# NVIDIA/retinanet-examples

Hardware: AMD Instinct MI355X
Metric: images/sec end-to-end (incl. decode+NMS), RN50FPN 800px bs=8 (higher is better)
Workload: dtype bf16; 1 GPU; ResNet50FPN bf16 inference, bs=8 per GPU at 800x1280, HIP decode x5 + NMS; global_batch=8, parallelism=replicas x1 (no data-path collective), entry=Model.forward (eval), postproc=fused

## Files before the change

include/odtk_hip.h:

```cpp
#ifndef ODTK_HIP_H
#define ODTK_HIP_H

#include <stddef.h>
#include <stdint.h>

#ifdef __cplusplus
extern "C" {
#endif

#define ODTK_OK                0
#define ODTK_ERR_INVALID      -1
#define ODTK_ERR_WORKSPACE    -2
#define ODTK_ERR_HIP          -3
#define ODTK_ERR_UNSUPPORTED  -4

#define ODTK_MAX_LEVELS    6
#define ODTK_MAX_ANCHORS   32
#define ODTK_ATSS_MAX_TOPK 16
#define ODTK_MAX_TOP_N     16384
#define ODTK_MAX_NMS_COUNT 7680
#define ODTK_MAX_NMS_COUNT_SCRATCH (1 << 22)
#define ODTK_MAX_NMS_DETECTIONS 2048

#define ODTK_F32   0
// ... 174 lines not shown
                       const odtk_image_t *images, int max_pixels, const void *src, size_t src_bytes, const int32_t *tables,
                       size_t tables_len, const void *norm_table, void *out, int height, int width, int dtype, void *workspace,
                       size_t workspace_bytes, void *stream);
int odtk_gemm_init(const char *hipblaslt_path);
size_t odtk_gemm_plan_export(char *text, size_t capacity);
int odtk_gemm_plan_import(const char *text);
int odtk_gemm_plan_pin_misses(void);
#define ODTK_GEMM_ORIGIN_TIMED   0
#define ODTK_GEMM_ORIGIN_PINNED  1
#define ODTK_GEMM_ORIGIN_CAPTURE 2
int odtk_debug_gemm_candidates(size_t m, int n, int k, int dtype, int relu, int residual, size_t workspace_size,
                               int *indices, int capacity);
void odtk_gemm_plan_clear(void);
int odtk_gemm_last_solution(int *origin);
int odtk_gemm_bias_act(void *y, const void *x, const void *w, const float *bias, const void *residual,
                       size_t m, int n, int k, int dtype, int relu,
                       void *workspace, size_t workspace_size, void *stream);
int odtk_bottleneck_seam(void *out, void *z, const void *y2, const void *skip, const void *w3, const float *b3, const void *w1,
                         const float *b1, size_t m, int c_in, int c_mid, int c_next, int dtype, void *stream);

int odtk_tower_conv3x3(void *y, const void *x, const void *w, const void *bias, int batch_size, int height, int width, int c_in,
                       int c_out, int dtype, int relu, void *stream);
int odtk_debug_tower_conv_variant(int variant);

int odtk_snap_to_anchors(int batch_size, const float *targets, int n_max, const float *anchors,
                         int num_anchors, int num_classes, int height, int width, int stride,
                         float iou_background, float iou_foreground,
                         float *cls_target, float *box_target, float *depth, void *stream);

typedef struct odtk_snap_level {
  const float *anchors;
  float *cls_target;
  float *box_target;
  float *depth;
  int32_t height, width, stride, pad_;
} odtk_snap_level_t;
int odtk_snap_to_anchors_levels(int batch_size, const float *targets, int n_max, int n_levels,
                                const odtk_snap_level_t *levels, int num_anchors, int num_classes,
                                float iou_background, float iou_foreground, void *stream);

int odtk_atss_assign_levels(int batch_size, const float *targets, int n_max, int n_levels,
                            const odtk_snap_level_t *levels, int num_anchors, int num_classes, int topk,
                            void *workspace, size_t workspace_size, void *stream);

struct odtk_loss_level;
int odtk_tal_assign_levels(int batch_size, const float *targets, int n_max, int n_levels,
// ... 124 lines not shown
```

retinanet-examples_amd/csrc/engine.hip:

```cpp
#include <cstring>

#include "runtime.hpp"
#include "epilogue.hpp"
#include "gemm_lt.hpp"
#include "seam.hpp"
#include "tower_conv.hpp"

namespace {

constexpr int kStreamCapMax = 65536, kStreamWideBit = 1 << 20;
std::atomic<int> g_stream_tuning{0};

inline int stream_tuning() { return g_stream_tuning.load(std::memory_order_relaxed); }

inline uint64_t stream_grid(uint64_t blocks, uint64_t own_cap, int tuning) {
  const uint64_t cap = (tuning & (kStreamWideBit - 1)) ? static_cast<uint64_t>(tuning & (kStreamWideBit - 1)) : own_cap;
  return blocks > cap ? cap : blocks;
}

struct BiasActPlan {
  bool fast;
  uint32_t blocks;
  uint32_t vpr;
  uint64_t n_vec;
// ... 66 lines not shown

template <typename T, int N2>
int seam_launch(const void *y2, const void *skip, const void *w3, const float *b3, const void *w1, const float *b1, void *out, void *z,
                uint64_t m, hipStream_t stream) {
  constexpr size_t lds = odtk::seam_lds_bytes<N2>();
  const int rc = allow_dynamic_lds(reinterpret_cast<const void *>(&odtk::bottleneck_seam_kernel<T, N2>), lds, "bottleneck_seam_kernel LDS");
  if (rc != ODTK_OK) return rc;
  int device = 0, cus = 0;
  ODTK_HIP_TRY(hipGetDevice(&device));
  ODTK_HIP_TRY(hipDeviceGetAttribute(&cus, hipDeviceAttributeMultiprocessorCount, device));
  constexpr uint64_t per_group = odtk::kSeamThreads / 64 * 32;
  uint64_t blocks = (m + per_group - 1) / per_group;
  const uint64_t resident = static_cast<uint64_t>(cus > 0 ? cus : 1) * (160 * 1024 / lds);
  if (blocks > resident) blocks = resident;
  timed_launch(ODTK_KERNEL_SEAM, odtk::bottleneck_seam_kernel<T, N2>, dim3(static_cast<unsigned>(blocks)), dim3(odtk::kSeamThreads), lds, stream,
               static_cast<const uint16_t *>(y2), static_cast<const uint16_t *>(skip), static_cast<const uint16_t *>(w3), b3,
               static_cast<const uint16_t *>(w1), b1, static_cast<uint16_t *>(out), static_cast<uint16_t *>(z), m);
  ODTK_HIP_TRY(hipGetLastError());
  return ODTK_OK;
}

std::atomic<int> g_tower_variant{1};

template <typename T, bool kRelu, int kForm>
int tower_conv_launch(void *y, const void *x, const void *w, const void *bias, uint32_t m, uint32_t height, uint32_t width, bool remap,
                      hipStream_t stream) {
  const int rc = allow_dynamic_lds(reinterpret_cast<const void *>(&odtk::tower_conv3x3_kernel<T, kRelu, kForm>), odtk::tower::kLdsBytes,
                                   "tower_conv3x3_kernel LDS");
  if (rc != ODTK_OK) return rc;
  const uint32_t tiles = (m + odtk::tower::kTilePixels - 1) / odtk::tower::kTilePixels;
  timed_launch(ODTK_KERNEL_TOWER_CONV, odtk::tower_conv3x3_kernel<T, kRelu, kForm>, dim3(tiles), dim3(odtk::tower::kThreads),
               odtk::tower::kLdsBytes, stream, static_cast<const unsigned char *>(x), static_cast<const unsigned char *>(w),
               static_cast<const uint16_t *>(bias), static_cast<unsigned char *>(y), m, height, width, odtk::fastdiv_make(width),
               odtk::fastdiv_make(height * width), remap ? 1u : 0u);
  ODTK_HIP_TRY(hipGetLastError());
  return ODTK_OK;
}

template <typename T>
int tower_conv_typed(void *y, const void *x, const void *w, const void *bias, uint32_t m, uint32_t h, uint32_t wd, bool relu, int variant,
                     hipStream_t s) {
  const bool remap = variant & 1;
  if (variant & 2) return relu ? tower_conv_launch<T, true, 0>(y, x, w, bias, m, h, wd, remap, s) : tower_conv_launch<T, false, 0>(y, x, w, bias, m, h, wd, remap, s);
  return relu ? tower_conv_launch<T, true, 1>(y, x, w, bias, m, h, wd, remap, s) : tower_conv_launch<T, false, 1>(y, x, w, bias, m, h, wd, remap, s);
}

}

extern "C" {

int odtk_debug_tower_conv_variant(int variant) {
  if (variant < -1 || variant > 3) return ODTK_ERR_INVALID;
  return variant < 0 ? g_tower_variant.load() : g_tower_variant.exchange(variant);
}

int odtk_debug_stream_tuning(int grid_cap, int pool_wide_index) {
  if (grid_cap < -1 || grid_cap > kStreamCapMax || pool_wide_index < -1 || pool_wide_index > 1) return ODTK_ERR_INVALID;
  int was = g_stream_tuning.load(std::memory_order_relaxed), now;
  do {
    now = (grid_cap < 0 ? was & (kStreamWideBit - 1) : grid_cap) | (pool_wide_index < 0 ? was & kStreamWideBit : pool_wide_index ? kStreamWideBit : 0);
  } while (!g_stream_tuning.compare_exchange_weak(was, now, std::memory_order_relaxed));
  return ODTK_OK;
}

int odtk_debug_stream_tuning_get(int out[2]) {
  if (!out) return ODTK_ERR_INVALID;
  const int tuning = stream_tuning();
// ... 11 lines not shown
  out[1] = p.blocks;
  out[2] = static_cast<unsigned>(p.stride);
  out[3] = p.trips > 0xffffffffull ? 0xffffffffu : static_cast<unsigned>(p.trips);
  return ODTK_OK;
}

int odtk_tower_conv3x3(void *y, const void *x, const void *w, const void *bias, int batch_size, int height, int width, int c_in, int c_out,
                       int dtype, int relu, void *stream) {
  if (!y || !x || !w || !bias || batch_size <= 0 || height <= 0 || width <= 0 || c_in <= 0 || c_out <= 0) return ODTK_ERR_INVALID;
  if (y == x) return ODTK_ERR_INVALID;
  if (dtype != ODTK_BF16 && dtype != ODTK_F16) return ODTK_ERR_UNSUPPORTED;
  if (c_in != static_cast<int>(odtk::tower::kChannels) || c_out != static_cast<int>(odtk::tower::kChannels)) return ODTK_ERR_UNSUPPORTED;
  if ((reinterpret_cast<uintptr_t>(y) | reinterpret_cast<uintptr_t>(x) | reinterpret_cast<uintptr_t>(w) | reinterpret_cast<uintptr_t>(bias)) & 15u)
    return ODTK_ERR_INVALID;
  const uint64_t m = static_cast<uint64_t>(batch_size) * static_cast<uint64_t>(height) * static_cast<uint64_t>(width);
  if (m * odtk::tower::kPixelBytes >= (1ull << 31)) return ODTK_ERR_UNSUPPORTED;
  hipStream_t s = static_cast<hipStream_t>(stream);
  const int variant = g_tower_variant.load(std::memory_order_relaxed);
  if (dtype == ODTK_BF16)
    return tower_conv_typed<odtk::BF16>(y, x, w, bias, static_cast<uint32_t>(m), static_cast<uint32_t>(height), static_cast<uint32_t>(width),
                                        relu != 0, variant, s);
  return tower_conv_typed<odtk::F16>(y, x, w, bias, static_cast<uint32_t>(m), static_cast<uint32_t>(height), static_cast<uint32_t>(width),
                                      relu != 0, variant, s);
}

int odtk_bottleneck_seam(void *out, void *z, const void *y2, const void *skip, const void *w3, const float *b3, const void *w1,
                         const float *b1, size_t m, int c_in, int c_mid, int c_next, int dtype, void *stream) {
  if (!out || !z || !y2 || !skip || !w3 || !b3 || !w1 || !b1 || c_in <= 0 || c_mid <= 0 || c_next <= 0) return ODTK_ERR_INVALID;
  if (out == z || out == y2 || out == skip || z == y2 || z == skip) return ODTK_ERR_INVALID;
  if (dtype != ODTK_BF16 && dtype != ODTK_F16) return ODTK_ERR_UNSUPPORTED;
  if (c_in != odtk::kSeamCin || c_mid != odtk::kSeamCmid || (c_next != 64 && c_next != 128)) return ODTK_ERR_UNSUPPORTED;
  if ((reinterpret_cast<uintptr_t>(out) | reinterpret_cast<uintptr_t>(z) | reinterpret_cast<uintptr_t>(y2) | reinterpret_cast<uintptr_t>(skip) |
       reinterpret_cast<uintptr_t>(w3) | reinterpret_cast<uintptr_t>(w1)) & 15u)
    return ODTK_ERR_INVALID;
  if ((reinterpret_cast<uintptr_t>(b3) | reinterpret_cast<uintptr_t>(b1)) & 3u) return ODTK_ERR_INVALID;
  if (m > (1ull << 40)) return ODTK_ERR_INVALID;
  if (m == 0) return ODTK_OK;
  hipStream_t s = static_cast<hipStream_t>(stream);
  if (dtype == ODTK_BF16)
    return c_next == 64 ? seam_launch<odtk::BF16, 64>(y2, skip, w3, b3, w1, b1, out, z, m, s)
                        : seam_launch<odtk::BF16, 128>(y2, skip, w3, b3, w1, b1, out, z, m, s);
  return c_next == 64 ? seam_launch<odtk::F16, 64>(y2, skip, w3, b3, w1, b1, out, z, m, s)
                      : seam_launch<odtk::F16, 128>(y2, skip, w3, b3, w1, b1, out, z, m, s);
}

int odtk_bias_act(void *y, const float *bias, const void *residual, size_t n_pixels, int channels, int dtype,
// ... 147 lines not shown
```

retinanet-examples_amd/csrc/tower_conv.hpp:

```cpp
#pragma once

#include "common.hpp"
#include "seam.hpp"
#include "tower_conv_layout.hpp"

namespace odtk {

typedef float tower_f32x4 __attribute__((ext_vector_type(4)));

__device__ __attribute__((aligned(16))) uint32_t tower_zero_block[4];

template <typename T>
__device__ __forceinline__ tower_f32x4 tower_mfma(vuint4 a, vuint4 b, tower_f32x4 c) {
  if constexpr (std::is_same_v<T, BF16>)
    return __builtin_amdgcn_mfma_f32_16x16x32_bf16(__builtin_bit_cast(seam_bf16x8, a), __builtin_bit_cast(seam_bf16x8, b), c, 0, 0, 0);
  else
    return __builtin_amdgcn_mfma_f32_16x16x32_f16(__builtin_bit_cast(seam_f16x8, a), __builtin_bit_cast(seam_f16x8, b), c, 0, 0, 0);
}

template <typename T>
__device__ __forceinline__ seam_f32x16 tower_mfma32(vuint4 a, vuint4 b, seam_f32x16 c) {
  if constexpr (std::is_same_v<T, BF16>)
    return __builtin_amdgcn_mfma_f32_32x32x16_bf16(__builtin_bit_cast(seam_bf16x8, a), __builtin_bit_cast(seam_bf16x8, b), c, 0, 0, 0);
  else
    return __builtin_amdgcn_mfma_f32_32x32x16_f16(__builtin_bit_cast(seam_f16x8, a), __builtin_bit_cast(seam_f16x8, b), c, 0, 0, 0);
}

__device__ __forceinline__ void tower_glds16(const unsigned char *src, unsigned char *lds_wave_base) {
  __builtin_amdgcn_global_load_lds((const __attribute__((address_space(1))) void *)src,
                                   (__attribute__((address_space(3))) void *)lds_wave_base, 16, 0, 0);
}

template <typename T, bool kRelu, int kForm>
__global__ __launch_bounds__(tower::kThreads) void tower_conv3x3_kernel(const unsigned char *__restrict__ x, const unsigned char *__restrict__ w,
                                                                        const uint16_t *__restrict__ bias, unsigned char *__restrict__ y,
                                                                        uint32_t m, uint32_t height, uint32_t width, FastDiv by_w,
                                                                        FastDiv by_hw, uint32_t remap) {
  using namespace tower;
  extern __shared__ __attribute__((aligned(1024))) unsigned char tower_lds[];

  const uint32_t tid = threadIdx.x, lane = tid & 63u;
  const uint32_t wave = __builtin_amdgcn_readfirstlane(tid >> 6);
  uint32_t tile = blockIdx.x;
  if (remap) {
    const uint32_t nwg = gridDim.x, q = nwg >> 3, r = nwg & 7u, xcd = tile & 7u;
    tile = (xcd < r ? xcd * (q + 1u) : r * (q + 1u) + (xcd - r) * q) + (tile >> 3);
  }

  const uint32_t chunk_bytes = piece_chunk(tid) * 16u;
  int32_t a_base[4];
  uint32_t a_mask[4];
#pragma unroll
  for (uint32_t i = 0; i < 4; ++i) {
    const uint32_t p = tile * kTilePixels + piece_row(i, tid);
    a_base[i] = 0;
    a_mask[i] = 0u;
    if (p < m) {
      const Pixel px = pixel_of(p, by_w, by_hw);
      a_base[i] = static_cast<int32_t>(p * kPixelBytes + chunk_bytes);
      a_mask[i] = tap_mask(px.y, px.x, height, width);
// ... 17 lines not shown
  };

  const uint32_t wr = wave >> 2, wc = wave & 3u;
  using Acc = std::conditional_t<kForm == 0, tower_f32x4[4][8], seam_f32x16[2][4]>;
  Acc acc;
  if constexpr (kForm == 0) {
#pragma unroll
    for (int n = 0; n < 4; ++n)
#pragma unroll
      for (int b = 0; b < 8; ++b) acc[n][b] = tower_f32x4{0.0f, 0.0f, 0.0f, 0.0f};
  } else {
#pragma unroll
    for (int n = 0; n < 2; ++n)
#pragma unroll
      for (int b = 0; b < 4; ++b)
#pragma unroll
        for (int e = 0; e < 16; ++e) acc[n][b][e] = 0.0f;
  }
  uint32_t f[4];
  if constexpr (kForm == 0) {
    f[0] = frag_addr(0, 0, lane); f[1] = frag_addr(0, 1, lane); f[2] = f[3] = 0u;
  } else {
#pragma unroll
    for (uint32_t s = 0; s < 4; ++s) f[s] = frag32_addr(0, s, lane);
  }
  const uint32_t x_frag = wr * 128u * kRowBytes, w_frag = kOperandBytes + wc * 64u * kRowBytes;

  auto compute = [&](const unsigned char *buf) {
    if constexpr (kForm == 0) {
#pragma unroll
      for (uint32_t kk = 0; kk < 2; ++kk) {
        vuint4 wf[4], xf[8];
#pragma unroll
        for (uint32_t n = 0; n < 4; ++n) wf[n] = *reinterpret_cast<const vuint4 *>(buf + w_frag + n * 16u * kRowBytes + f[kk]);
#pragma unroll
        for (uint32_t b = 0; b < 8; ++b) xf[b] = *reinterpret_cast<const vuint4 *>(buf + x_frag + b * 16u * kRowBytes + f[kk]);
#pragma unroll
        for (uint32_t n = 0; n < 4; ++n)
#pragma unroll
          for (uint32_t b = 0; b < 8; ++b) acc[n][b] = tower_mfma<T>(wf[n], xf[b], acc[n][b]);
      }
    } else {
#pragma unroll
      for (uint32_t s = 0; s < 4; ++s) {
        vuint4 wf[2], xf[4];
#pragma unroll
        for (uint32_t n = 0; n < 2; ++n) wf[n] = *reinterpret_cast<const vuint4 *>(buf + w_frag + n * 32u * kRowBytes + f[s]);
// ... 33 lines not shown
      }
  } else {
#pragma unroll
    for (uint32_t n = 0; n < 2; ++n)
#pragma unroll
      for (uint32_t b = 0; b < 4; ++b)
#pragma unroll
        for (uint32_t g = 0; g < 4; ++g) {
          const uint32_t at = out_addr(acc32_pixel(wr * 4u + b, lane), acc32_channel(wc * 2u + n, lane, 4u * g));
          uint2 v;
          v.x = seam_pack2<T>(acc[n][b][4 * g], acc[n][b][4 * g + 1]);
          v.y = seam_pack2<T>(acc[n][b][4 * g + 2], acc[n][b][4 * g + 3]);
          *reinterpret_cast<uint2 *>(tower_lds + at) = v;
        }
  }
  __syncthreads();
  const uint32_t pixel0 = tid >> 5, chunk = out_chunk(pixel0, tid & 31u);
  float bias8[8];
  {
    const vuint4 bv = *reinterpret_cast<const vuint4 *>(bias + chunk * 8u);
#pragma unroll
    for (int e = 0; e < 8; ++e) bias8[e] = seam_unpack<T>(bv[e >> 1], e & 1);
  }
#pragma unroll 4
  for (uint32_t it = 0; it < 16; ++it) {
    const uint32_t pixel = it * 16u + pixel0, p = tile * kTilePixels + pixel;
    const vuint4 v = *reinterpret_cast<const vuint4 *>(tower_lds + (it * kThreads + tid) * 16u);
    vuint4 r;
#pragma unroll
    for (int d = 0; d < 4; ++d) {
      float o[2];
#pragma unroll
      for (int e = 0; e < 2; ++e) {
        const float s = seam_unpack<T>(v[d], e) + bias8[2 * d + e];
        o[e] = kRelu ? (s > 0.0f ? s : (s != s ? s : 0.0f)) : s;
      }
      r[d] = seam_pack2<T>(o[0], o[1]);
    }
    if (p < m) *reinterpret_cast<vuint4 *>(y + static_cast<size_t>(p) * kPixelBytes + chunk * 16u) = r;
  }
}

}
```

retinanet-examples_amd/csrc/tower_conv_layout.hpp:

```cpp
#pragma once

#include "fastdiv.hpp"

namespace odtk {
namespace tower {

constexpr uint32_t kThreads = 512;
constexpr uint32_t kTilePixels = 256, kChannels = 256, kBK = 64, kTaps = 9;
constexpr uint32_t kKTiles = kTaps * kChannels / kBK;
constexpr uint32_t kRowBytes = kBK * 2, kOperandBytes = 256 * kRowBytes;
constexpr uint32_t kBufferBytes = 2 * kOperandBytes;
constexpr uint32_t kLdsBytes = 2 * kBufferBytes;
constexpr uint32_t kPixelBytes = kChannels * 2;

ODTK_HD uint32_t swizzle(uint32_t row, uint32_t chunk) { return chunk ^ ((row >> 1) & 7u); }

ODTK_HD uint32_t piece_dst(uint32_t i, uint32_t tid) { return (i * kThreads + tid) * 16u; }
ODTK_HD uint32_t piece_wave_base(uint32_t i, uint32_t wave) { return (i * kThreads + wave * 64u) * 16u; }
ODTK_HD uint32_t piece_row(uint32_t i, uint32_t tid) { return i * 64u + (tid >> 3); }
ODTK_HD uint32_t piece_chunk(uint32_t tid) { return swizzle(tid >> 3, tid & 7u); }

ODTK_HD uint32_t frag_row(uint32_t block, uint32_t lane) { return block * 16u + (lane & 15u); }
ODTK_HD uint32_t frag_chunk(uint32_t kk, uint32_t lane) { return kk * 4u + (lane >> 4); }
ODTK_HD uint32_t frag_addr(uint32_t block, uint32_t kk, uint32_t lane) {
  const uint32_t row = frag_row(block, lane);
  return row * kRowBytes + (swizzle(row, frag_chunk(kk, lane)) << 4);
}

ODTK_HD uint32_t frag32_row(uint32_t block, uint32_t lane) { return block * 32u + (lane & 31u); }
ODTK_HD uint32_t frag32_chunk(uint32_t step, uint32_t lane) { return (step >> 1) * 4u + 2u * (lane >> 5) + (step & 1u); }
ODTK_HD uint32_t frag32_addr(uint32_t block, uint32_t step, uint32_t lane) {
  const uint32_t row = frag32_row(block, lane);
  return row * kRowBytes + (swizzle(row, frag32_chunk(step, lane)) << 4);
}

ODTK_HD uint32_t ktile_tap(uint32_t kt) { return kt >> 2; }
ODTK_HD uint32_t ktile_channel(uint32_t kt) { return (kt & 3u) * kBK; }
ODTK_HD int32_t tap_pixel_offset(uint32_t tap, uint32_t width) {
  return (static_cast<int32_t>(tap / 3u) - 1) * static_cast<int32_t>(width) + (static_cast<int32_t>(tap % 3u) - 1);
}

struct Pixel { uint32_t n, y, x; };
ODTK_HD Pixel pixel_of(uint32_t p, const FastDiv &by_w, const FastDiv &by_hw) {
  Pixel q;
  uint32_t rem;
  q.n = fastdivmod(p, by_hw, &rem);
  q.y = fastdivmod(rem, by_w, &q.x);
  return q;
}

ODTK_HD uint32_t tap_mask(uint32_t y, uint32_t x, uint32_t height, uint32_t width) {
  const uint32_t rows = (y > 0u ? 1u : 0u) | 2u | (y + 1u < height ? 4u : 0u);
  const uint32_t cols = (x > 0u ? 1u : 0u) | 2u | (x + 1u < width ? 4u : 0u);
  uint32_t mask = 0u;
  for (uint32_t kh = 0; kh < 3u; ++kh)
    if ((rows >> kh) & 1u) mask |= cols << (3u * kh);
  return mask;
}

ODTK_HD uint32_t out_chunk(uint32_t pixel, uint32_t chunk) { return (chunk & ~7u) | ((chunk ^ pixel) & 7u); }
ODTK_HD uint32_t out_addr(uint32_t pixel, uint32_t channel) {
  return pixel * kPixelBytes + out_chunk(pixel, channel >> 3) * 16u + (channel & 4u) * 2u;
}
ODTK_HD uint32_t acc_channel(uint32_t nb, uint32_t lane, uint32_t reg) { return nb * 16u + (lane >> 4) * 4u + reg; }
ODTK_HD uint32_t acc_pixel(uint32_t mb, uint32_t lane) { return mb * 16u + (lane & 15u); }
ODTK_HD uint32_t acc32_channel(uint32_t nb, uint32_t lane, uint32_t reg) { return nb * 32u + (reg & 3u) + 8u * (reg >> 2) + 4u * (lane >> 5); }
ODTK_HD uint32_t acc32_pixel(uint32_t mb, uint32_t lane) { return mb * 32u + (lane & 31u); }

}
}
```

retinanet-examples_amd/odtk/_C.py:

```python
import ctypes
import threading
import os

import torch

_LIB_PATH = os.environ.get('ODTK_HIP_LIBRARY') or os.path.join(os.path.dirname(os.path.abspath(__file__)), 'libodtk_hip.so')

OK, ERR_INVALID, ERR_WORKSPACE, ERR_HIP, ERR_UNSUPPORTED = 0, -1, -2, -3, -4
F32, BF16, F16 = 0, 1, 2
FLAG_ROTATED, FLAG_LOGITS, FLAG_ROTATED_NMS_FIXED_ANGLE = 1, 2, 4
MAX_LEVELS, MAX_ANCHORS, MAX_TOP_N, MAX_NMS_COUNT, MAX_NMS_COUNT_SCRATCH = 6, 32, 16384, 7680, 1 << 22
MAX_CONCAT_PARTS = 8
MAX_TILES = 64
MAX_OPTIM_TENSORS, OPTIM_CHUNK = 64, 4096
SOFT_NMS_LINEAR, SOFT_NMS_GAUSSIAN = 1, 2
MATRIX_NMS_LINEAR, MATRIX_NMS_GAUSSIAN = 1, 2
MAX_MATRIX_NMS_PRE = 4096
ATSS_MAX_TOPK = 16
BOX_LOSS_IOU, BOX_LOSS_GIOU, BOX_LOSS_DIOU = 1, 2, 3
BOX_LOSS_KINDS = {'iou': BOX_LOSS_IOU, 'giou': BOX_LOSS_GIOU, 'diou': BOX_LOSS_DIOU}
ROTATED_BOX_LOSS_PROBIOU, ROTATED_BOX_LOSS_KLD = 1, 2
ROTATED_BOX_LOSS_KINDS = {'probiou': ROTATED_BOX_LOSS_PROBIOU, 'kld': ROTATED_BOX_LOSS_KLD}
CLS_LOSS_QFL, CLS_LOSS_VFL = 1, 2
CLS_LOSS_KINDS = {'qfl': CLS_LOSS_QFL, 'vfl': CLS_LOSS_VFL}
# ... 158 lines not shown
    'odtk_soft_nms': (ctypes.c_int, [ctypes.c_int, _vpp, _vpp, ctypes.c_int, _sz, ctypes.c_int, ctypes.c_float, ctypes.c_int,
                                     ctypes.c_float, ctypes.c_float, ctypes.c_uint32, _vp, _sz, _vp]),
    'odtk_matrix_nms': (ctypes.c_int, [ctypes.c_int, _vpp, _vpp, ctypes.c_int, _sz, ctypes.c_int, ctypes.c_int, ctypes.c_int,
                                       ctypes.c_float, ctypes.c_float, ctypes.c_uint32, _vp, _sz, _vp]),
    'odtk_box_vote': (ctypes.c_int, [ctypes.c_int, _vpp, _vp, _vp, _sz, ctypes.c_int, ctypes.c_float, ctypes.c_uint32, _vp]),
    'odtk_concat_candidates': (ctypes.c_int, [ctypes.c_int, ctypes.c_int, ctypes.POINTER(Candidates), _vpp, ctypes.c_uint32, _vp]),
    'odtk_tile_images': (ctypes.c_int, [_vp, _vp] + [ctypes.c_int] * 7 + [ctypes.POINTER(Tile), ctypes.c_int, ctypes.c_int, _vp]),
    'odtk_merge_tile_candidates': (ctypes.c_int, [ctypes.c_int, ctypes.POINTER(Tile), _vpp, _vpp, _sz] + [ctypes.c_int] * 6 +
                                   [ctypes.c_float, ctypes.c_uint32, _vp]),
    'odtk_gemm_init': (ctypes.c_int, [ctypes.c_char_p]),
    'odtk_gemm_plan_export': (ctypes.c_size_t, [ctypes.c_char_p, ctypes.c_size_t]),
    'odtk_gemm_plan_import': (ctypes.c_int, [ctypes.c_char_p]),
    'odtk_gemm_plan_pin_misses': (ctypes.c_int, []),
    'odtk_debug_gemm_candidates': (ctypes.c_int, [ctypes.c_size_t] + [ctypes.c_int] * 5 + [ctypes.c_size_t, ctypes.POINTER(ctypes.c_int),
                                                  ctypes.c_int]),
    'odtk_gemm_plan_clear': (None, []),
    'odtk_gemm_last_solution': (ctypes.c_int, [ctypes.POINTER(ctypes.c_int)]),
    'odtk_gemm_bias_act': (ctypes.c_int, [ctypes.c_void_p, ctypes.c_void_p, ctypes.c_void_p, ctypes.c_void_p, ctypes.c_void_p,
                                          ctypes.c_size_t, ctypes.c_int, ctypes.c_int, ctypes.c_int, ctypes.c_int,
                                          ctypes.c_void_p, ctypes.c_size_t, ctypes.c_void_p]),
    'odtk_bottleneck_seam': (ctypes.c_int, [ctypes.c_void_p] * 8 + [ctypes.c_size_t] + [ctypes.c_int] * 4 + [ctypes.c_void_p]),
    'odtk_tower_conv3x3': (ctypes.c_int, [ctypes.c_void_p] * 4 + [ctypes.c_int] * 7 + [ctypes.c_void_p]),
    'odtk_debug_tower_conv_variant': (ctypes.c_int, [ctypes.c_int]),
    'odtk_profile_collect': (ctypes.c_int, [ctypes.POINTER(ctypes.c_double), ctypes.POINTER(ctypes.c_int)]),
}

KERNEL_NAMES = ('prefilter_scan_kernel', 'select_decode_kernel', 'nms_kernel', 'iou_pairs_kernel', 'bias_act_kernel',
                'snap_to_anchors_kernel', 'gemm_bias_act', 'retina_loss_kernel', 'select_hist_kernel', 'select_filter_kernel',
                'nms_first_round_kernel', 'rotated_sup_matrix_kernel', 'bias_act_maxpool_kernel', 'upsample_nearest2x_kernel',
                'stem_pack_kernel', 'loss_reduce_kernel', 'atss_stats_kernel', 'bottleneck_seam_kernel', 'tower_conv3x3_kernel')
traffic_count = False
traffic_bytes = {}


def _count(name, nbytes):
    if traffic_count:
        traffic_bytes[name] = traffic_bytes.get(name, 0) + int(nbytes)


_lib = None


def library():
    global _lib
    if _lib is None:
        if not os.path.isfile(_LIB_PATH):
# ... 994 lines not shown


def tower_conv3x3(x, weight, bias, relu=True):
    if not x.is_cuda or x.dim() != 4 or x.dtype not in (torch.bfloat16, torch.float16):
        raise RuntimeError('tower_conv3x3: x must be a 4-d CUDA tensor of bfloat16/float16')
    b, c, h, w = x.shape
    n = weight.shape[0]
    if (weight.dim() != 4 or tuple(weight.shape[1:]) != (c, 3, 3) or weight.dtype != x.dtype or weight.device != x.device
            or not weight.is_contiguous(memory_format=torch.channels_last)):
        raise RuntimeError('tower_conv3x3: weight must be a channels_last [Cout, %d, 3, 3] tensor of x.dtype' % c)
    if not x.is_contiguous(memory_format=torch.channels_last):
        raise RuntimeError('tower_conv3x3: x must be channels_last')
    if bias.dtype != x.dtype or bias.numel() != n or bias.device != x.device or not bias.is_contiguous():
        raise RuntimeError('tower_conv3x3: bias must be a dense vector of length Cout of x.dtype')
    y = torch.empty((b, n, h, w), dtype=x.dtype, device=x.device, memory_format=torch.channels_last)
    if y.numel() == 0:
        return y
    _launch(library().odtk_tower_conv3x3, 'tower_conv3x3', x.device, y.data_ptr(), x.data_ptr(), weight.data_ptr(), bias.data_ptr(),
            b, h, w, c, n, _DTYPES[x.dtype], 1 if relu else 0)
    _count('tower_conv3x3_kernel', (x.numel() + y.numel()) * x.element_size())
    return y


_CONV_LIB_PATH = os.path.join(os.path.dirname(os.path.abspath(__file__)), 'libodtk_conv.so')
_conv_lib = []


def conv_library():
    if not _conv_lib:
        lib = None
        if os.path.isfile(_CONV_LIB_PATH) and not os.environ.get('ODTK_NO_CONV_LIBRARY'):
            lib = ctypes.CDLL(_CONV_LIB_PATH)
            lib.odtk_conv_bias_act.restype = ctypes.c_int
            lib.odtk_conv_bias_act.argtypes = [ctypes.c_void_p] * 4 + [ctypes.c_int] * 13 + [ctypes.c_void_p]
            lib.odtk_conv_bias_act_pads.restype = ctypes.c_int
            lib.odtk_conv_bias_act_pads.argtypes = [ctypes.c_void_p] * 4 + [ctypes.c_int] * 15 + [ctypes.c_void_p]
            lib.odtk_conv_bias_act_strided.restype = ctypes.c_int
            lib.odtk_conv_bias_act_strided.argtypes = ([ctypes.c_void_p] * 4 + [ctypes.c_int] * 13 + [ctypes.c_longlong] * 6 +
                                                       [ctypes.c_int] * 2 + [ctypes.c_void_p])
            lib.odtk_conv_last_plan.restype = ctypes.c_char_p
            lib.odtk_conv_last_plan.argtypes = []
            lib.odtk_conv_instance_count.restype = ctypes.c_int
            lib.odtk_conv_instance_count.argtypes = [ctypes.c_int]
            lib.odtk_conv_plan_export.restype = ctypes.c_size_t
            lib.odtk_conv_plan_export.argtypes = [ctypes.c_char_p, ctypes.c_size_t]
            lib.odtk_conv_plan_import.restype = ctypes.c_int
# ... 240 lines not shown
```

retinanet-examples_amd/odtk/fused.py:

```python
import hashlib
import json
import os
import threading

import torch
import torch.nn as nn
import torch.nn.functional as F

from . import _C
from . import box as box_ops
from .backbones.resnet import BasicBlock, Bottleneck


_PLAN_LOCK = threading.Lock()
_TLS = threading.local()


def _planning():
    return getattr(_TLS, 'planning', False)


def _key_str(key):
    kind, shape = ('only', key[1:]) if key and key[0] == 'only' else ('act', key)
    return kind + ':' + 'x'.join(str(int(v)) for v in shape)
# ... 44 lines not shown
    shelf_w, row_y, row_h, cursor = None, 0, 0, shelf_x
    for h, w in shapes[1:]:
        if shelf_w is None:
            shelf_w = w
        elif cursor + w > shelf_x + shelf_w and row_y + row_h + gutter + h <= height:
            row_y, row_h, cursor = row_y + row_h + gutter, 0, shelf_x
        origins.append((row_y, cursor))
        shelf_w = max(shelf_w, cursor + w - shelf_x)
        row_h = max(row_h, h)
        cursor += w + gutter
    return ((max(y + h for (y, _), (h, _) in zip(origins, shapes)), max(x + w for (_, x), (_, w) in zip(origins, shapes))), origins)


def _window(x):
    return (x.dim() == 4 and x.shape[1] > 1 and x.stride(1) == 1 and x.stride(3) >= x.shape[1]
            and all(v % 8 == 0 for v in (x.stride(0), x.stride(2), x.stride(3))))


class _Conv(nn.Module):

    use_conv_library = True
    tower_conv = os.environ.get('ODTK_TOWER_CONV', '1') != '0'
    tower_min_pixels = 100000
    route_mode = os.environ.get('ODTK_CONV_ROUTE', 'auto')

    def __init__(self, conv, bn=None, relu=False, dtype=torch.bfloat16):
        super().__init__()
        w, b = fold_conv_bn(conv, bn)
        self.register_buffer('weight', w.to(dtype).contiguous(memory_format=torch.channels_last))
        self.register_buffer('bias', b.contiguous())
        self.register_buffer('bias_lp', b.to(dtype).contiguous())
        self.stride, self.padding, self.relu, self.groups = conv.stride, conv.padding, relu, conv.groups
        self.pointwise = (tuple(conv.kernel_size) == (1, 1) and tuple(conv.padding) == (0, 0) and conv.groups == 1
                          and tuple(conv.dilation) == (1, 1))
        self.library_ok = (not self.pointwise and conv.groups == 1 and tuple(conv.dilation) == (1, 1)
                           and dtype in (torch.bfloat16, torch.float16) and w.shape[1] % 8 == 0)
        self.strided_ok = (self.pointwise and tuple(conv.stride) != (1, 1) and dtype in (torch.bfloat16, torch.float16)
                           and w.shape[1] % 8 == 0)
        self.tower_ok = (tuple(w.shape) == (256, 256, 3, 3) and tuple(conv.stride) == (1, 1) and tuple(conv.padding) == (1, 1)
                         and tuple(conv.dilation) == (1, 1) and conv.groups == 1 and dtype in (torch.bfloat16, torch.float16))
        self.zero_bias = None
        self.learned = {}
        self.route = {}

    def conv_only(self, x):
        library = False
        if (self.library_ok and _Conv.use_conv_library and x.is_cuda and x.is_contiguous(memory_format=torch.channels_last)
                and _C.conv_available()):
            key = ('only',) + tuple(x.shape)
            if self.zero_bias is None:
                self.zero_bias = torch.zeros_like(self.bias_lp)
            library = self._routed(key, 'only', x, self._miopen_only, self._library_only)
        if library and self._tower_takes(x):
            try:
                return _C.tower_conv3x3(x, self.weight, self.zero_bias, False)
            except RuntimeError:
                pass
        if library:
            try:
                return self._library_only(x)
            except RuntimeError:
                self.route[key] = (False, float('inf'), 0.0)
        return self._miopen_only(x)

    def _tower_takes(self, x, residual=None):
        return (self.tower_ok and self.tower_conv and residual is None and x.is_cuda and x.dim() == 4 and x.dtype == self.weight.dtype
                and x.is_contiguous(memory_format=torch.channels_last)
                and x.shape[0] * x.shape[2] * x.shape[3] >= self.tower_min_pixels)

    def on_view(self, x, only=False):
        if x.is_contiguous(memory_format=torch.channels_last):
            return self.conv_only(x) if only else self(x)
        if self.library_ok and _Conv.use_conv_library and x.is_cuda and _window(x) and _C.conv_available():
            if only and self.zero_bias is None:
                self.zero_bias = torch.zeros_like(self.bias_lp)
            key = (('only',) + tuple(x.shape)) if only else tuple(x.shape)
            two, one = (self._miopen_only, self._library_only) if only else (self._two_pass, self._one_pass)
            if self._routed(key, 'only' if only else 'act', x, two, one):
                try:
                    return self._library_only(x) if only else self._one_pass(x)
                except RuntimeError:
                    pass
        x = x.contiguous(memory_format=torch.channels_last)
        return self.conv_only(x) if only else self(x)

    def _torch(self, x, residual=None):
        y = F.conv2d(x, self.weight, None, self.stride, self.padding, groups=self.groups) + self.bias.to(x.dtype).view(1, -1, 1, 1)
        if residual is not None:
            y = y + residual
        return (F.relu(y) if self.relu else y).contiguous(memory_format=torch.channels_last)

# ... 140 lines not shown
        if not self.supports(model):
            raise ValueError('FusedRetinaNet supports a single ResNet-FPN backbone')
        fpn = next(iter(model.backbones.values()))
        net = fpn.features
        self.dtype = dtype
        self.model = [model]
        self.stem = _Conv(net.conv1, net.bn1, True, dtype)
        self.stem_s2d = None
        c1 = net.conv1
        if (tuple(c1.kernel_size), tuple(c1.stride), tuple(c1.padding), c1.in_channels, c1.groups) == ((7, 7), (2, 2), (3, 3), 3, 1) \
                and dtype in (torch.bfloat16, torch.float16):
            w = self.stem.weight.float()
            w4 = stem_space_to_depth_weights(w)
            self.register_buffer('stem_w4', w4.to(dtype).contiguous(memory_format=torch.channels_last))
            self.register_buffer('stem_zero_bias', torch.zeros(w.shape[0], dtype=dtype, device=w.device))
            self.stem_s2d = {}
        self.stem_learned = False
        self.layers = nn.ModuleList([nn.ModuleList([_Block(b, dtype) for b in layer])
                                     for layer in (net.layer1, net.layer2, net.layer3, net.layer4)])
        blocks = [b for layer in self.layers for b in layer]
        self._seams = {a: b for a, b in zip(blocks, blocks[1:]) if a.seam_to(b, dtype)}
        self.seam_fusion = os.environ.get('ODTK_SEAM_FUSION', '1') != '0'
        self._tower_conv = _Conv.tower_conv
        self.outputs = list(net.outputs)
        self.lateral = nn.ModuleList([_Conv(fpn.lateral3, None, False, dtype), _Conv(fpn.lateral4, None, False, dtype),
                                      _Conv(fpn.lateral5, None, False, dtype)])
        self.smooth = nn.ModuleList([_Conv(fpn.smooth3, None, False, dtype), _Conv(fpn.smooth4, None, False, dtype),
                                     _Conv(fpn.smooth5, None, False, dtype)])
        self.pyramid6 = _Conv(fpn.pyramid6, None, False, dtype)
        self.pyramid7 = _Conv(fpn.pyramid7, None, False, dtype)

        def head(seq):
            convs = [m for m in seq if isinstance(m, nn.Conv2d)]
            return nn.ModuleList([_Conv(c, None, i + 1 < len(convs), dtype) for i, c in enumerate(convs)])

        self.cls_head = head(model.cls_head)
        self.box_head = head(model.box_head)
        self.level_streams = True
        self.pyramid_canvas = os.environ.get('ODTK_PYRAMID_CANVAS', '1') != '0'
        self._streams = None
        self.tower_plan = 0
        self._planned = set()
        self._loaded_geometries = set()
        self._plan_file_seen = False
        self.libraries_taken = None
        self.max_plans = 4
        self._graphs = {}
        self._thresholds = {}
        self.max_graphs = 8

    @property
    def tower_conv(self):
        return self._tower_conv

    @tower_conv.setter
    def tower_conv(self, on):
        self._tower_conv = bool(on)
        for mod in self.modules():
            if isinstance(mod, _Conv):
                mod.tower_conv = self._tower_conv

    def _stem_direct(self, x):
        x = x.to(self.dtype).contiguous(memory_format=torch.channels_last)
        return self.stem.conv_then_pool(x)

    def _stem_packed(self, x):
        xs = _C.stem_pack(x, self.dtype)
        y = _C.conv_bias_act(xs, self.stem_w4, self.stem_zero_bias, 1, ((2, 1), (2, 1)), False)
        return _C.bias_act_maxpool(y, self.stem.bias, self.stem.relu)

    def _stem(self, x):
        if (self.stem_s2d is not None and _Conv.use_conv_library and x.is_cuda and x.dim() == 4 and x.shape[1] == 3
                and x.shape[2] % 2 == 0 and x.shape[3] % 2 == 0 and x.dtype in _C._DTYPES and _C.conv_available()
                and (x.is_contiguous() or x.is_contiguous(memory_format=torch.channels_last))):
            key = (tuple(x.shape), x.dtype, x.is_contiguous())
            route = self.stem_s2d.get(key)
            if route is None and _Conv.route_mode != 'auto':
                route = self.stem_s2d[key] = (_Conv.route_mode == 'library', None, None)
            if route is None and _planning() and not torch.cuda.is_current_stream_capturing():
                route = self.stem_s2d[key] = self.stem._measure(x, self._stem_direct, self._stem_packed)
                self.stem_learned = route[0]
            if route[0] if route is not None else self.stem_learned:
                try:
# ... 49 lines not shown
        if first.is_cuda and ((first.shape[1] * first.element_size()) % 16 or len(feats) - 1 > _C.MAX_LEVELS
                              or not all(t.is_contiguous(memory_format=torch.channels_last) for t in feats[1:])):
            return None
        return gutter

    def _canvas_towers(self, feats, gutter, last_bias):
        shapes = [(t.shape[2], t.shape[3]) for t in feats]
        (height, width), origins = pyramid_canvas_layout(shapes, gutter)
        rects = [(y, x, h, w) for (y, x), (h, w) in zip(origins, shapes)]
        if feats[0].is_cuda:
            canvas = _C.canvas_pack(feats, rects, height, width)
            mask = None
        else:
            first = feats[0]
            canvas = torch.zeros((first.shape[0], first.shape[1], height, width), dtype=first.dtype).contiguous(memory_format=torch.channels_last)
            mask = torch.ones((1, 1, height, width), dtype=torch.bool)
            for t, (y, x, h, w) in zip(feats, rects):
                canvas[:, :, y:y + h, x:x + w] = t
                mask[:, :, y:y + h, x:x + w] = False
        out = []
        for head in (self.cls_head, self.box_head):
            t = canvas
            for j, c in enumerate(head[:-1]):
                t = c(t)
                if gutter and j + 2 < len(head):
                    t = _C.canvas_clear_(t, rects) if t.is_cuda else t.masked_fill_(mask, 0)
            last = head[-1]
            views = [t[:, :, y:y + h, x:x + w] for y, x, h, w in rects]
            out.append([last.on_view(v, not last_bias) for v in views])
        return list(zip(*out))

    def _towers(self, feats, last_bias, level_streams=None):
        out = [None] * len(feats)

        def level(t):
            if last_bias:
                return self._run(self.cls_head, t), self._run(self.box_head, t)
            return (self.cls_head[-1].conv_only(self._run(self.cls_head[:-1], t)),
                    self.box_head[-1].conv_only(self._run(self.box_head[:-1], t)))

        def unit(i):
            if i == 'canvas':
                out[1:] = self._canvas_towers(feats[1:], gutter, last_bias)
                return out[1:]
            out[i] = level(feats[i])
            return [out[i]]

        gutter = self._canvas_gutter(feats)
        if level_streams is None:
# ... 25 lines not shown
                e = torch.cuda.Event()
                e.record(stream)
                done.append(e)
        for i in mine:
            unit(i)
        for e in done:
            main.wait_event(e)
        return [o[0] for o in out], [o[1] for o in out]

    def heads(self, x):
        with torch.autocast(x.device.type, enabled=False):
            return self._towers(self.features(x), True)

    def heads_without_last_bias(self, x):
        with torch.autocast(x.device.type, enabled=False):
            cls, box = self._towers(self.features(x), False)
        return cls, box, self.cls_head[-1].bias, self.box_head[-1].bias

    @torch.no_grad()
    def replay(self, x):
        m = self.model[0]
        bias = self.cls_head[-1].bias
        key = (tuple(x.shape), x.dtype, x.device, x.is_contiguous(memory_format=torch.channels_last),
               m.threshold, m.top_n, m.nms, m.detections, self.level_streams, self.tower_plan, self.pyramid_canvas, self.seam_fusion, self.tower_conv, bias.data_ptr(), bias._version,
               tuple(sorted(m.soft_nms.items())) if getattr(m, 'soft_nms', None) is not None else None,
               getattr(m, 'box_voting', None),
               tuple(sorted(m.matrix_nms.items())) if getattr(m, 'matrix_nms', None) is not None else None)
        if getattr(m, 'tta', None) is not None:
            raise RuntimeError('FusedRetinaNet.replay is not available with Model.tta (two passes of the engine)')
        if getattr(m, 'tile', None) is not None:
            raise RuntimeError('FusedRetinaNet.replay is not available with Model.tile (several passes of the engine)')
        entry = self._graphs.get(key)
        if entry is None:
            static_x = torch.empty_like(x)
            static_x.copy_(x)
            side = torch.cuda.Stream(x.device)
            side.wait_stream(torch.cuda.current_stream(x.device))
            with torch.cuda.stream(side):
                for _ in range(2):
                    self.forward(static_x)
            torch.cuda.current_stream(x.device).wait_stream(side)
            graph = torch.cuda.CUDAGraph()
            with torch.cuda.graph(graph):
                out = self.forward(static_x)
            while len(self._graphs) >= self.max_graphs:
                self._graphs.pop(next(iter(self._graphs)))
            entry = self._graphs[key] = (graph, static_x, out, tuple(self._thresholds.values()))
# ... 133 lines not shown
```

Before: 1305 images/s.

## Run canvas tower convs through custom 3x3 kernel with fused gutter masking

Adds a canvas_conv3x3 entry point that runs the packed pyramid-canvas head-tower convolutions through the custom tower 3x3 kernel. It adds a new fragment form (frag64) and an optional rectangle mask that zeroes gutter pixels in the epilogue, using a wave ballot. This replaces the separate canvas_clear_ pass and lets canvases smaller than the usual tower threshold (down to 48000 pixels) use the custom kernel. The cost is extra per-tile rectangle tests and a new, less-tested fragment layout. It falls back to the old path on any error.

```diff
diff --git a/include/odtk_hip.h b/include/odtk_hip.h
--- a/include/odtk_hip.h
+++ b/include/odtk_hip.h
@@ -220,6 +220,8 @@
 int odtk_tower_conv3x3(void *y, const void *x, const void *w, const void *bias, int batch_size, int height, int width, int c_in,
                        int c_out, int dtype, int relu, void *stream);
 int odtk_debug_tower_conv_variant(int variant);
+int odtk_canvas_conv3x3(void *y, const void *x, const void *w, const void *bias, int batch_size, int height, int width, int c_in,
+                        int c_out, int dtype, int relu, int form, const int *rects, int n_rects, void *stream);
 
 int odtk_snap_to_anchors(int batch_size, const float *targets, int n_max, const float *anchors,
                          int num_anchors, int num_classes, int height, int width, int stride,
diff --git a/retinanet-examples_amd/csrc/engine.hip b/retinanet-examples_amd/csrc/engine.hip
--- a/retinanet-examples_amd/csrc/engine.hip
+++ b/retinanet-examples_amd/csrc/engine.hip
@@ -112,17 +112,19 @@
 
 std::atomic<int> g_tower_variant{1};
 
-template <typename T, bool kRelu, int kForm>
+static_assert(odtk::tower::kMaxRects == ODTK_MAX_LEVELS, "the kernel's rectangle table holds one entry per pyramid level");
+
+template <typename T, bool kRelu, int kForm, bool kMasked = false>
 int tower_conv_launch(void *y, const void *x, const void *w, const void *bias, uint32_t m, uint32_t height, uint32_t width, bool remap,
-                      hipStream_t stream) {
-  const int rc = allow_dynamic_lds(reinterpret_cast<const void *>(&odtk::tower_conv3x3_kernel<T, kRelu, kForm>), odtk::tower::kLdsBytes,
-                                   "tower_conv3x3_kernel LDS");
+                      hipStream_t stream, const odtk::tower::Rects &rects = odtk::tower::Rects{}) {
+  const int rc = allow_dynamic_lds(reinterpret_cast<const void *>(&odtk::tower_conv3x3_kernel<T, kRelu, kForm, kMasked>),
+                                   odtk::tower::kLdsBytes, "tower_conv3x3_kernel LDS");
   if (rc != ODTK_OK) return rc;
   const uint32_t tiles = (m + odtk::tower::kTilePixels - 1) / odtk::tower::kTilePixels;
-  timed_launch(ODTK_KERNEL_TOWER_CONV, odtk::tower_conv3x3_kernel<T, kRelu, kForm>, dim3(tiles), dim3(odtk::tower::kThreads),
+  timed_launch(ODTK_KERNEL_TOWER_CONV, odtk::tower_conv3x3_kernel<T, kRelu, kForm, kMasked>, dim3(tiles), dim3(odtk::tower::kThreads),
                odtk::tower::kLdsBytes, stream, static_cast<const unsigned char *>(x), static_cast<const unsigned char *>(w),
                static_cast<const uint16_t *>(bias), static_cast<unsigned char *>(y), m, height, width, odtk::fastdiv_make(width),
-               odtk::fastdiv_make(height * width), remap ? 1u : 0u);
+               odtk::fastdiv_make(height * width), remap ? 1u : 0u, rects);
   ODTK_HIP_TRY(hipGetLastError());
   return ODTK_OK;
 }
@@ -133,6 +135,16 @@
   const bool remap = variant & 1;
   if (variant & 2) return relu ? tower_conv_launch<T, true, 0>(y, x, w, bias, m, h, wd, remap, s) : tower_conv_launch<T, false, 0>(y, x, w, bias, m, h, wd, remap, s);
   return relu ? tower_conv_launch<T, true, 1>(y, x, w, bias, m, h, wd, remap, s) : tower_conv_launch<T, false, 1>(y, x, w, bias, m, h, wd, remap, s);
+}
+
+template <typename T, bool kRelu>
+int canvas_conv_typed(void *y, const void *x, const void *w, const void *bias, uint32_t m, uint32_t h, uint32_t wd, int form, bool masked,
+                      const odtk::tower::Rects &rects, bool remap, hipStream_t s) {
+  if (form == 2)
+    return masked ? tower_conv_launch<T, kRelu, 2, true>(y, x, w, bias, m, h, wd, remap, s, rects)
+                  : tower_conv_launch<T, kRelu, 2, false>(y, x, w, bias, m, h, wd, remap, s);
+  return masked ? tower_conv_launch<T, kRelu, 1, true>(y, x, w, bias, m, h, wd, remap, s, rects)
+                : tower_conv_launch<T, kRelu, 1, false>(y, x, w, bias, m, h, wd, remap, s);
 }
 
 }
@@ -190,6 +202,33 @@
                                         relu != 0, variant, s);
   return tower_conv_typed<odtk::F16>(y, x, w, bias, static_cast<uint32_t>(m), static_cast<uint32_t>(height), static_cast<uint32_t>(width),
                                       relu != 0, variant, s);
+}
+
+int odtk_canvas_conv3x3(void *y, const void *x, const void *w, const void *bias, int batch_size, int height, int width, int c_in, int c_out,
+                        int dtype, int relu, int form, const int *rects, int n_rects, void *stream) {
+  if (!y || !x || !w || !bias || batch_size <= 0 || height <= 0 || width <= 0 || c_in <= 0 || c_out <= 0) return ODTK_ERR_INVALID;
+  if (y == x || (form != 1 && form != 2) || n_rects < 0 || n_rects > ODTK_MAX_LEVELS || (n_rects > 0 && !rects)) return ODTK_ERR_INVALID;
+  if (dtype != ODTK_BF16 && dtype != ODTK_F16) return ODTK_ERR_UNSUPPORTED;
+  if (c_in != static_cast<int>(odtk::tower::kChannels) || c_out != static_cast<int>(odtk::tower::kChannels)) return ODTK_ERR_UNSUPPORTED;
+  if ((reinterpret_cast<uintptr_t>(y) | reinterpret_cast<uintptr_t>(x) | reinterpret_cast<uintptr_t>(w) | reinterpret_cast<uintptr_t>(bias)) & 15u)
+    return ODTK_ERR_INVALID;
+  odtk::tower::Rects table{};
+  for (int l = 0; l < n_rects; ++l) {
+    const int y0 = rects[4 * l], x0 = rects[4 * l + 1], h = rects[4 * l + 2], wd = rects[4 * l + 3];
+    if (y0 < 0 || x0 < 0 || h <= 0 || wd <= 0 || y0 > height - h || x0 > width - wd) return ODTK_ERR_INVALID;
+    table.y0[l] = static_cast<uint32_t>(y0); table.x0[l] = static_cast<uint32_t>(x0);
+    table.h[l] = static_cast<uint32_t>(h); table.w[l] = static_cast<uint32_t>(wd);
+  }
+  const uint64_t m = static_cast<uint64_t>(batch_size) * static_cast<uint64_t>(height) * static_cast<uint64_t>(width);
+  if (m * odtk::tower::kPixelBytes >= (1ull << 31)) return ODTK_ERR_UNSUPPORTED;
+  hipStream_t s = static_cast<hipStream_t>(stream);
+  const bool remap = g_tower_variant.load(std::memory_order_relaxed) & 1, masked = n_rects > 0;
+  const uint32_t pixels = static_cast<uint32_t>(m), h = static_cast<uint32_t>(height), wd = static_cast<uint32_t>(width);
+  if (dtype == ODTK_BF16)
+    return relu ? canvas_conv_typed<odtk::BF16, true>(y, x, w, bias, pixels, h, wd, form, masked, table, remap, s)
+                : canvas_conv_typed<odtk::BF16, false>(y, x, w, bias, pixels, h, wd, form, masked, table, remap, s);
+  return relu ? canvas_conv_typed<odtk::F16, true>(y, x, w, bias, pixels, h, wd, form, masked, table, remap, s)
+              : canvas_conv_typed<odtk::F16, false>(y, x, w, bias, pixels, h, wd, form, masked, table, remap, s);
 }
 
 int odtk_bottleneck_seam(void *out, void *z, const void *y2, const void *skip, const void *w3, const float *b3, const void *w1,
diff --git a/retinanet-examples_amd/csrc/tower_conv.hpp b/retinanet-examples_amd/csrc/tower_conv.hpp
--- a/retinanet-examples_amd/csrc/tower_conv.hpp
+++ b/retinanet-examples_amd/csrc/tower_conv.hpp
@@ -31,11 +31,11 @@
                                    (__attribute__((address_space(3))) void *)lds_wave_base, 16, 0, 0);
 }
 
-template <typename T, bool kRelu, int kForm>
+template <typename T, bool kRelu, int kForm, bool kMasked = false>
 __global__ __launch_bounds__(tower::kThreads) void tower_conv3x3_kernel(const unsigned char *__restrict__ x, const unsigned char *__restrict__ w,
                                                                         const uint16_t *__restrict__ bias, unsigned char *__restrict__ y,
                                                                         uint32_t m, uint32_t height, uint32_t width, FastDiv by_w,
-                                                                        FastDiv by_hw, uint32_t remap) {
+                                                                        FastDiv by_hw, uint32_t remap, const tower::Rects rects) {
   using namespace tower;
   extern __shared__ __attribute__((aligned(1024))) unsigned char tower_lds[];
 
@@ -99,7 +99,7 @@
     f[0] = frag_addr(0, 0, lane); f[1] = frag_addr(0, 1, lane); f[2] = f[3] = 0u;
   } else {
 #pragma unroll
-    for (uint32_t s = 0; s < 4; ++s) f[s] = frag32_addr(0, s, lane);
+    for (uint32_t s = 0; s < 4; ++s) f[s] = kForm == 2 ? frag64_addr(0, s, lane) : frag32_addr(0, s, lane);
   }
   const uint32_t x_frag = wr * 128u * kRowBytes, w_frag = kOperandBytes + wc * 64u * kRowBytes;
 
@@ -179,6 +179,11 @@
 #pragma unroll
     for (int e = 0; e < 8; ++e) bias8[e] = seam_unpack<T>(bv[e >> 1], e & 1);
   }
+  uint32_t inside = 0xffffffffu;
+  if constexpr (kMasked) {
+    const Pixel px = pixel_of(tile * kTilePixels + mask_lane_pixel(wave, lane), by_w, by_hw);
+    inside = static_cast<uint32_t>(__builtin_amdgcn_ballot_w64(in_rects(rects, px.y, px.x)));
+  }
 #pragma unroll 4
   for (uint32_t it = 0; it < 16; ++it) {
     const uint32_t pixel = it * 16u + pixel0, p = tile * kTilePixels + pixel;
@@ -194,6 +199,9 @@
       }
       r[d] = seam_pack2<T>(o[0], o[1]);
     }
+    if constexpr (kMasked) {
+      if (!((inside >> mask_bit(it, tid)) & 1u)) r = vuint4{0u, 0u, 0u, 0u};
+    }
     if (p < m) *reinterpret_cast<vuint4 *>(y + static_cast<size_t>(p) * kPixelBytes + chunk * 16u) = r;
   }
 }
diff --git a/retinanet-examples_amd/csrc/tower_conv_layout.hpp b/retinanet-examples_amd/csrc/tower_conv_layout.hpp
--- a/retinanet-examples_amd/csrc/tower_conv_layout.hpp
+++ b/retinanet-examples_amd/csrc/tower_conv_layout.hpp
@@ -34,6 +34,12 @@
   return row * kRowBytes + (swizzle(row, frag32_chunk(step, lane)) << 4);
 }
 
+ODTK_HD uint32_t frag64_chunk(uint32_t step, uint32_t lane) { return 4u * (lane >> 5) + step; }
+ODTK_HD uint32_t frag64_addr(uint32_t block, uint32_t step, uint32_t lane) {
+  const uint32_t row = frag32_row(block, lane);
+  return row * kRowBytes + (swizzle(row, frag64_chunk(step, lane)) << 4);
+}
+
 ODTK_HD uint32_t ktile_tap(uint32_t kt) { return kt >> 2; }
 ODTK_HD uint32_t ktile_channel(uint32_t kt) { return (kt & 3u) * kBK; }
 ODTK_HD int32_t tap_pixel_offset(uint32_t tap, uint32_t width) {
@@ -58,6 +64,17 @@
   return mask;
 }
 
+constexpr uint32_t kMaxRects = 6;
+struct Rects { uint32_t y0[kMaxRects], x0[kMaxRects], h[kMaxRects], w[kMaxRects]; };
+ODTK_HD bool in_rects(const Rects &r, uint32_t y, uint32_t x) {
+  bool inside = false;
+  for (uint32_t l = 0; l < kMaxRects; ++l)
+    inside = inside || (y - r.y0[l] < r.h[l] && x - r.x0[l] < r.w[l]);
+  return inside;
+}
+ODTK_HD uint32_t mask_lane_pixel(uint32_t wave, uint32_t lane) { return ((lane & 31u) >> 1) * 16u + 2u * wave + (lane & 1u); }
+ODTK_HD uint32_t mask_bit(uint32_t it, uint32_t tid) { return 2u * it + ((tid >> 5) & 1u); }
+
 ODTK_HD uint32_t out_chunk(uint32_t pixel, uint32_t chunk) { return (chunk & ~7u) | ((chunk ^ pixel) & 7u); }
 ODTK_HD uint32_t out_addr(uint32_t pixel, uint32_t channel) {
   return pixel * kPixelBytes + out_chunk(pixel, channel >> 3) * 16u + (channel & 4u) * 2u;
diff --git a/retinanet-examples_amd/odtk/_C.py b/retinanet-examples_amd/odtk/_C.py
--- a/retinanet-examples_amd/odtk/_C.py
+++ b/retinanet-examples_amd/odtk/_C.py
@@ -204,6 +204,8 @@
     'odtk_bottleneck_seam': (ctypes.c_int, [ctypes.c_void_p] * 8 + [ctypes.c_size_t] + [ctypes.c_int] * 4 + [ctypes.c_void_p]),
     'odtk_tower_conv3x3': (ctypes.c_int, [ctypes.c_void_p] * 4 + [ctypes.c_int] * 7 + [ctypes.c_void_p]),
     'odtk_debug_tower_conv_variant': (ctypes.c_int, [ctypes.c_int]),
+    'odtk_canvas_conv3x3': (ctypes.c_int, [ctypes.c_void_p] * 4 + [ctypes.c_int] * 8 + [ctypes.POINTER(ctypes.c_int), ctypes.c_int,
+                                                                                            ctypes.c_void_p]),
     'odtk_profile_collect': (ctypes.c_int, [ctypes.POINTER(ctypes.c_double), ctypes.POINTER(ctypes.c_int)]),
 }
 
@@ -1244,6 +1246,30 @@
     return y
 
 
+def canvas_conv3x3(x, weight, bias, relu=True, form=2, rects=()):
+    if not x.is_cuda or x.dim() != 4 or x.dtype not in (torch.bfloat16, torch.float16):
+        raise RuntimeError('canvas_conv3x3: x must be a 4-d CUDA tensor of bfloat16/float16')
+    b, c, h, w = x.shape
+    n = weight.shape[0]
+    if (weight.dim() != 4 or tuple(weight.shape[1:]) != (c, 3, 3) or weight.dtype != x.dtype or weight.device != x.device
+            or not weight.is_contiguous(memory_format=torch.channels_last)):
+        raise RuntimeError('canvas_conv3x3: weight must be a channels_last [Cout, %d, 3, 3] tensor of x.dtype' % c)
+    if not x.is_contiguous(memory_format=torch.channels_last):
+        raise RuntimeError('canvas_conv3x3: x must be channels_last')
+    if bias.dtype != x.dtype or bias.numel() != n or bias.device != x.device or not bias.is_contiguous():
+        raise RuntimeError('canvas_conv3x3: bias must be a dense vector of length Cout of x.dtype')
+    flat = [int(v) for r in rects for v in r]
+    if len(flat) != 4 * len(rects):
+        raise RuntimeError('canvas_conv3x3: a rectangle is (y0, x0, height, width)')
+    y = torch.empty((b, n, h, w), dtype=x.dtype, device=x.device, memory_format=torch.channels_last)
+    if y.numel() == 0:
+        return y
+    _launch(library().odtk_canvas_conv3x3, 'canvas_conv3x3', x.device, y.data_ptr(), x.data_ptr(), weight.data_ptr(), bias.data_ptr(),
+            b, h, w, c, n, _DTYPES[x.dtype], 1 if relu else 0, int(form), (ctypes.c_int * max(len(flat), 1))(*flat), len(rects))
+    _count('tower_conv3x3_kernel', (x.numel() + y.numel()) * x.element_size())
+    return y
+
+
 _CONV_LIB_PATH = os.path.join(os.path.dirname(os.path.abspath(__file__)), 'libodtk_conv.so')
 _conv_lib = []
 
diff --git a/retinanet-examples_amd/odtk/fused.py b/retinanet-examples_amd/odtk/fused.py
--- a/retinanet-examples_amd/odtk/fused.py
+++ b/retinanet-examples_amd/odtk/fused.py
@@ -90,6 +90,8 @@
     use_conv_library = True
     tower_conv = os.environ.get('ODTK_TOWER_CONV', '1') != '0'
     tower_min_pixels = 100000
+    canvas_conv = os.environ.get('ODTK_CANVAS_CONV', '1') != '0'
+    canvas_min_pixels = 48000
     route_mode = os.environ.get('ODTK_CONV_ROUTE', 'auto')
 
     def __init__(self, conv, bn=None, relu=False, dtype=torch.bfloat16):
@@ -135,6 +137,19 @@
         return (self.tower_ok and self.tower_conv and residual is None and x.is_cuda and x.dim() == 4 and x.dtype == self.weight.dtype
                 and x.is_contiguous(memory_format=torch.channels_last)
                 and x.shape[0] * x.shape[2] * x.shape[3] >= self.tower_min_pixels)
+
+    def on_canvas(self, x, rects):
+        if not (self.tower_ok and self.canvas_conv and self.tower_conv and x.is_cuda and x.dim() == 4 and x.dtype == self.weight.dtype
+                and x.is_contiguous(memory_format=torch.channels_last)
+                and x.shape[0] * x.shape[2] * x.shape[3] >= self.canvas_min_pixels):
+            return None
+        if not (self.library_ok and _Conv.use_conv_library and _C.conv_available()
+                and self._routed(tuple(x.shape), 'act', x, self._two_pass, self._one_pass)):
+            return None
+        try:
+            return _C.canvas_conv3x3(x, self.weight, self.bias_lp, self.relu, 2, rects)
+        except RuntimeError:
+            return None
 
     def on_view(self, x, only=False):
         if x.is_contiguous(memory_format=torch.channels_last):
@@ -321,6 +336,7 @@
         self._seams = {a: b for a, b in zip(blocks, blocks[1:]) if a.seam_to(b, dtype)}
         self.seam_fusion = os.environ.get('ODTK_SEAM_FUSION', '1') != '0'
         self._tower_conv = _Conv.tower_conv
+        self._canvas_conv = _Conv.canvas_conv
         self.outputs = list(net.outputs)
         self.lateral = nn.ModuleList([_Conv(fpn.lateral3, None, False, dtype), _Conv(fpn.lateral4, None, False, dtype),
                                       _Conv(fpn.lateral5, None, False, dtype)])
@@ -358,6 +374,17 @@
         for mod in self.modules():
             if isinstance(mod, _Conv):
                 mod.tower_conv = self._tower_conv
+
+    @property
+    def canvas_conv(self):
+        return self._canvas_conv
+
+    @canvas_conv.setter
+    def canvas_conv(self, on):
+        self._canvas_conv = bool(on)
+        for mod in self.modules():
+            if isinstance(mod, _Conv):
+                mod.canvas_conv = self._canvas_conv
 
     def _stem_direct(self, x):
         x = x.to(self.dtype).contiguous(memory_format=torch.channels_last)
@@ -453,9 +480,13 @@
         for head in (self.cls_head, self.box_head):
             t = canvas
             for j, c in enumerate(head[:-1]):
-                t = c(t)
-                if gutter and j + 2 < len(head):
-                    t = _C.canvas_clear_(t, rects) if t.is_cuda else t.masked_fill_(mask, 0)
+                clear = bool(gutter) and j + 2 < len(head)
+                y = c.on_canvas(t, rects if clear else ())
+                if y is None:
+                    y = c(t)
+                    if clear:
+                        y = _C.canvas_clear_(y, rects) if y.is_cuda else y.masked_fill_(mask, 0)
+                t = y
             last = head[-1]
             views = [t[:, :, y:y + h, x:x + w] for y, x, h, w in rects]
             out.append([last.on_view(v, not last_bias) for v in views])
@@ -527,7 +558,7 @@
         m = self.model[0]
         bias = self.cls_head[-1].bias
         key = (tuple(x.shape), x.dtype, x.device, x.is_contiguous(memory_format=torch.channels_last),
-               m.threshold, m.top_n, m.nms, m.detections, self.level_streams, self.tower_plan, self.pyramid_canvas, self.seam_fusion, self.tower_conv, bias.data_ptr(), bias._version,
+               m.threshold, m.top_n, m.nms, m.detections, self.level_streams, self.tower_plan, self.pyramid_canvas, self.seam_fusion, self.tower_conv, self.canvas_conv, bias.data_ptr(), bias._version,
                tuple(sorted(m.soft_nms.items())) if getattr(m, 'soft_nms', None) is not None else None,
                getattr(m, 'box_voting', None),
                tuple(sorted(m.matrix_nms.items())) if getattr(m, 'matrix_nms', None) is not None else None)
```

After: 1327 images/s (median of 6 runs). 1.6% higher.
